# anonymousauthors001/SGS-GNN

Measured on AMD Instinct MI355X. Metric: sampled edges/sec + training steps/sec, Reddit hybrid 20% sparsity, higher is better.
Workload: dtype f32

## Files before the change

include/sgs_hip.h:

```cpp
#ifndef SGS_HIP_H_
#define SGS_HIP_H_

#include <stddef.h>
#include <stdint.h>

#ifdef __cplusplus
extern "C" {
#endif

#define SGS_ABI_VERSION 1

#define SGS_OK 0
#define SGS_EINVAL (-1)
#define SGS_EWORKSPACE (-2)
#define SGS_EHIP (-3)

typedef void* sgs_stream_t;

int sgs_abi_version(void);
const char* sgs_last_error(void);

int sgs_rng_set_epoch_buffer(const uint64_t* epoch_dev);
int sgs_exp_noise(uint64_t seed, uint64_t stream_id, int64_t E, float* noise, sgs_stream_t stream);
int sgs_dropout_keep(uint64_t seed, uint32_t site, int64_t rows, int64_t cols, float p, uint8_t* keep,
// ... 111 lines not shown
                          float* Hn, sgs_stream_t stream);
int sgs_gcn_norm_bwd_edge(const float* gw_hat, const float* gloop, int64_t n_edges, int64_t N, const float* dis,
                          const int32_t* loop_eid, const int64_t* edge_index, const float* Hn, float* dw,
                          sgs_stream_t stream);

#define SGS_ACT_NONE 0
#define SGS_ACT_RELU 1
#define SGS_ACT_RELU_DROPOUT 2
int sgs_spmm_csr(const float* X, int64_t N, int64_t D, int64_t nnz, const int32_t* ptr, const int32_t* col, const float* val,
                 const float* diag, const float* bias, int act, float p_drop, uint64_t seed, uint32_t site, float* Y,
                 sgs_stream_t stream);

int sgs_sddmm_csr(const float* A, const float* B, int64_t N, int64_t D, int64_t nnz, const int32_t* ptr, const int32_t* col,
                  const int32_t* eid, float* g, float* gdiag, sgs_stream_t stream);

int sgs_spmm_csr_variant(int64_t N, int64_t D, int64_t nnz, int aligned16);
int sgs_sddmm_csr_variant(int64_t N, int64_t D, int64_t nnz, int aligned16);

int sgs_spmm_long_rows_set(int on);
int sgs_spmm_long_rows_threshold(void);
int sgs_spmm_long_rows_active(int64_t N, int64_t D);

int sgs_act_bwd(const float* dY, const float* Y, int64_t n, int act, float p_drop, float* dZ, sgs_stream_t stream);
size_t sgs_colsum_workspace_bytes(int64_t N, int64_t D);
int sgs_colsum(const float* A, int64_t N, int64_t D, float* out, void* ws, size_t ws_bytes, sgs_stream_t stream);
int sgs_act_bwd_colsum(const float* dY, const float* Y, int64_t N, int64_t D, int act, float p_drop, float* dZ, float* colsum, void* ws,
                       size_t ws_bytes, sgs_stream_t stream);

int sgs_colsum_variant(int64_t N, int64_t D, int fused_act);

int sgs_gcn_pair_ok(int64_t N, int64_t nnz, int64_t D);
int sgs_spmm_csr_next(const float* X, int64_t N, int64_t D, int64_t nnz, const int32_t* ptr, const int32_t* col, const float* val,
                      const float* diag, const float* bias, int act, float p_drop, uint64_t seed, uint32_t site, const float* Wn, int64_t Dn,
                      float* Y, float* Z, sgs_stream_t stream);
int sgs_spmm_csr_bwd_prev(const float* dZ, int64_t N, int64_t D, int64_t nnz, const int32_t* ptr, const int32_t* col, const float* val,
                          const float* diag, const float* W, int64_t Dp, const float* Yp, int act, float p_drop, float* dX, float* dZp,
                          float* colsum, sgs_stream_t stream);

int sgs_gcn_dual_ok(int64_t N, int64_t nnz_a, int64_t nnz_b, int64_t D, int64_t Dn);
int sgs_spmm_csr_next_dual(const float* X, int64_t N, int64_t D, const float* bias, int act, float p_drop, uint32_t site, const float* Wn,
                           int64_t Dn, int64_t nnz_a, const int32_t* ptr_a, const int32_t* col_a, const float* val_a, const float* diag_a,
                           uint64_t seed_a, float* Y_a, float* Z_a, int64_t nnz_b, const int32_t* ptr_b, const int32_t* col_b,
                           const float* val_b, const float* diag_b, uint64_t seed_b, float* Y_b, float* Z_b, sgs_stream_t stream);
int sgs_spmm_csr_dual(const float* X_a, const float* X_b, int64_t N, int64_t D, const float* bias, int act, float p_drop, uint32_t site,
                      int64_t nnz_a, const int32_t* ptr_a, const int32_t* col_a, const float* val_a, const float* diag_a, uint64_t seed_a,
                      float* Y_a, int64_t nnz_b, const int32_t* ptr_b, const int32_t* col_b, const float* val_b, const float* diag_b,
                      uint64_t seed_b, float* Y_b, sgs_stream_t stream);

size_t sgs_edge_score_workspace_bytes(int64_t N, int64_t H, int64_t E);
int sgs_edge_score_hidden_supported(int64_t H);
int sgs_edge_score_get_variant(void);
int sgs_edge_score_get_bwd_variant(void);
void sgs_edge_score_set_bwd_variant(int variant);
int sgs_edge_score_bwd_tile(void);
void sgs_edge_score_set_variant(int variant);
int sgs_edge_score_fwd(const float* codes, const float* U, int64_t N, int64_t H, const int64_t* edge_index, int64_t E,
                       int64_t edge_id_offset, const float* W1, const float* b1, const float* w2, const float* b2,
                       float p_drop, uint64_t seed, uint32_t site, float* p_out, void* ws, size_t ws_bytes,
                       sgs_stream_t stream);
size_t sgs_edge_mates_workspace_bytes(int64_t n_edges);
int sgs_edge_mates(const int64_t* edge_index, int64_t n_edges, int64_t N, const int32_t* out_ptr, const int32_t* out_dst,
                   const int32_t* out_eid, int32_t* mate, void* ws, size_t ws_bytes, sgs_stream_t stream);
int sgs_edge_score_paired_supported(int64_t H);
int sgs_edge_score_fwd_paired(const float* codes, const float* U, int64_t N, int64_t H, const int64_t* edge_index, int64_t E,
                              int64_t edge_id_offset, const int32_t* canon, int64_t M, const int32_t* mate, const float* W1, const float* b1,
                              const float* w2, const float* b2, float p_drop, uint64_t seed, uint32_t site, float* p_out, void* ws,
                              size_t ws_bytes, sgs_stream_t stream);
int sgs_edge_score_bwd_core(const float* codes, const float* U, int64_t N, int64_t H, const int64_t* edge_index,
                            int64_t E, int64_t edge_id_offset, const int64_t* active_eid, int64_t n_active, const float* grad_p,
                            const float* W1, const float* b1, const float* w2, const float* b2, float p_drop,
                            uint64_t seed, uint32_t site, float* dv, float* hdz_part, float* dz, float* feat, void* ws,
                            size_t ws_bytes, sgs_stream_t stream);
int sgs_edge_score_bwd_dfeat_supported(int64_t H);
int sgs_edge_score_bwd_dfeat(const float* dv, int64_t n, int64_t H, const float* W1, float* dfeat, void* ws, size_t ws_bytes,
                             sgs_stream_t stream);

int sgs_edge_score_bwd_bits_supported(int64_t H);
int sgs_edge_score_fwd_mask(const float* codes, const float* U, int64_t N, int64_t H, const int64_t* edge_index, int64_t E,
                            int64_t edge_id_offset, const int32_t* canon, int64_t M, const int32_t* mate, const float* W1, const float* b1,
                            const float* w2, const float* b2, float p_drop, uint64_t seed, uint32_t site, float* p_out, uint32_t* maskbits,
                            void* ws, size_t ws_bytes, sgs_stream_t stream);
int sgs_edge_score_bwd_prep(const float* codes, int64_t N, int64_t H, const int64_t* edge_index, int64_t E, const int64_t* active_eid,
                            int64_t n_active, const float* grad_p, const float* p, const uint32_t* maskbits, float* dz, uint32_t* dvbits,
                            float* feat, sgs_stream_t stream);
int sgs_edge_score_dw2_from_parts(const float* W1, const float* T_raw, const float* U, const float* R_raw, const float* b1, const float* c_raw,
                                  int64_t N, int64_t H, float p_drop, float* dw2, sgs_stream_t stream);
int sgs_edge_score_probe_set(int stagger, int prio, uint32_t mode_mask);
int sgs_edge_score_probe_trace(unsigned long long* buf);
size_t sgs_edge_score_epd_workspace_bytes(int64_t H);
int sgs_edge_score_epd_fwd(const float* A, int64_t N, int64_t H, const int64_t* edge_index, int64_t E, int64_t edge_id_offset, const float* W1,
                           const float* b1, const float* w2, const float* b2, float p_hidden, uint64_t seed, uint32_t site, float p_ep,
                           uint64_t seed_x, uint32_t site_x, uint64_t seed_y, uint32_t site_y, float* p_out, void* ws, size_t ws_bytes,
                           sgs_stream_t stream);
int sgs_edge_score_epd_bwd_core(const float* A, int64_t N, int64_t H, const int64_t* edge_index, int64_t E, int64_t edge_id_offset,
                                const int64_t* active_eid, int64_t n_active, const float* grad_p, const float* W1, const float* b1, const float* w2,
                                const float* b2, float p_hidden, uint64_t seed, uint32_t site, float p_ep, uint64_t seed_x, uint32_t site_x,
                                uint64_t seed_y, uint32_t site_y, float* dv, float* hdz_part, float* dz, float* feat2, void* ws, size_t ws_bytes,
                                sgs_stream_t stream);
int sgs_edge_score_epd_reduce(const float* dfeat2, const float* A, int64_t N, int64_t H, const int32_t* in_ptr, const int32_t* in_src,
                              const int32_t* in_eid, const int32_t* out_ptr, const int32_t* out_dst, const int32_t* out_eid,
                              const int64_t* active_eid, int64_t edge_id_offset, float p_ep, uint64_t seed_x, uint32_t site_x, uint64_t seed_y,
                              uint32_t site_y, float* dA, sgs_stream_t stream);

int sgs_edge_score_bwd_prep_sd(const float* codes, int64_t N, int64_t H, const int64_t* edge_index, int64_t E, const int64_t* active_eid,
                               int64_t n_active, const float* grad_p, const float* p, const uint32_t* maskbits, float* dz, uint32_t* dvbits,
                               int32_t* sd, sgs_stream_t stream);
// ... 376 lines not shown
```

sgs-gnn_amd/csrc/edge_score.hip:

```cpp
#include <type_traits>

#include "sgs_common.h"
#include "endpoint_reduce.h"

namespace sgs {
namespace {

constexpr int kT = 256;
constexpr int kBM = 64;
constexpr int kBK = 16;
using f32x16 = __attribute__((ext_vector_type(16))) float;

__global__ void __launch_bounds__(kT) transpose_w1a(const float* __restrict__ W1, int H, float* __restrict__ WaT) {
    __shared__ float t[32][33];
    const int bx = blockIdx.x * 32, by = blockIdx.y * 32;
    const int tx = threadIdx.x & 31, ty = threadIdx.x >> 5;
    for (int r = ty; r < 32; r += 8) {
        const int h = by + r, k = bx + tx;
        t[r][tx] = (h < H && k < H) ? W1[static_cast<int64_t>(h) * 2 * H + k] : 0.f;
    }
    __syncthreads();
    for (int r = ty; r < 32; r += 8) {
        const int k = bx + r, h = by + tx;
        if (k < H && h < H) WaT[static_cast<int64_t>(k) * H + h] = t[tx][r];
// ... 890 lines not shown
    uint32_t p[3][4];
#pragma unroll
    for (int m = 0; m < 4; ++m) {
        float w0 = TRANSPOSED ? W1[static_cast<int64_t>(k0 + 2 * m) * 2 * H + h] : W1[static_cast<int64_t>(h) * 2 * H + k0 + 2 * m];
        float w1 = TRANSPOSED ? W1[static_cast<int64_t>(k0 + 2 * m + 1) * 2 * H + h] : W1[static_cast<int64_t>(h) * 2 * H + k0 + 2 * m + 1];
        if (TRANSPOSED && rowscale) { w0 *= rowscale[k0 + 2 * m] * scale; w1 *= rowscale[k0 + 2 * m + 1] * scale; }
        split3(w0, w1, p[0][m], p[1][m], p[2][m]);
    }
    uint4* o = Wp16 + (static_cast<int64_t>(kc) * NTl + t) * P * 64 + lane;
#pragma unroll
    for (int c = 0; c < P; ++c) o[c * 64] = make_uint4(p[c][0], p[c][1], p[c][2], p[c][3]);
}
inline int64_t pack_w1a_threads(int64_t H) { return (H / 16) * (H / 32) * 64; }

template <bool TRANSPOSED = false, int P = 3>
__global__ void __launch_bounds__(kT) pack_w1a_bf16x3(const float* __restrict__ W1, int H, uint4* __restrict__ Wp16,
                                                     const float* __restrict__ rowscale = nullptr, float scale = 1.f) {
    pack_w1a_bf16x3_one<TRANSPOSED, P>(static_cast<int64_t>(blockIdx.x) * kT + threadIdx.x, W1, H, Wp16, rowscale, scale);
}

template <bool SALU_MASK = false>
__device__ __forceinline__ uint32_t shift_in_bit(uint32_t acc, uint64_t mask) {
    uint32_t out;
    uint64_t carry_out;
    if constexpr (SALU_MASK) {
        asm("v_addc_co_u32_e64 %0, %1, %2, %2, %3" : "=v"(out), "=s"(carry_out) : "v"(acc), "s"(mask));
        return out;
    }
    asm("s_nop 1\n\tv_addc_co_u32_e64 %0, %1, %2, %2, %3" : "=v"(out), "=s"(carry_out) : "v"(acc), "s"(mask));
    return out;
}

#ifndef SGS_PHASE_PROBE
#define SGS_PHASE_PROBE 0
#endif
#if SGS_PHASE_PROBE
#define SGS_PHASE_STAMP(on, k, pre) do { if (on) asm volatile(pre "s_memtime %0\n\ts_waitcnt lgkmcnt(0)" : "=s"(pst[k]) :: "memory"); } while (0)
#define SGS_PHASE_BARRIER() do { if (!(a.prio & 4)) __syncthreads(); } while (0)
#else
#define SGS_PHASE_STAMP(on, k, pre) do { (void)(on); } while (0)
#define SGS_PHASE_BARRIER() __syncthreads()
#endif
#define SGS_STAMP(k) do { if (a.trace && tid == 0) a.trace[8 * blockIdx.x + (k)] = __builtin_readcyclecounter(); } while (0)

template <int NT, int NW, int MODE = 0, int NP = 3>
__global__ void __launch_bounds__(64 * NW, 8 / NW) edge_score_bf16x6_kernel(ScoreArgs a, const uint4* __restrict__ Wp16) {
    constexpr bool BWD = MODE == 1, FUSED = MODE == 5, GEMMB = MODE == 4 || MODE == 5, GEMM = MODE == 2 || GEMMB, PAIR = MODE == 3;
    constexpr bool ONE = NP == 1;
    static_assert(NP == 3 || (ONE && MODE != 1 && MODE != 2), "the one-piece form exists for MODEs 0, 3, 4 and 5");
    constexpr int H = 32 * NT;
    constexpr int NPH = H / 16;
    constexpr int CH = NT * NP * 64;
    constexpr int TH = 64 * NW;
    constexpr int SPT = CH / TH;
    static_assert(CH % TH == 0 && (ONE ? (SPT == 1 || SPT == 2) : (SPT == 3 || SPT == 6)), "unsupported shape");
    __shared__ uint4 wl[2][CH];
    __shared__ __attribute__((aligned(16))) float bw[2][H];
    const int tid = threadIdx.x, lane = tid & 63, wave = tid >> 6;
    const int kh = lane >> 5, l31 = lane & 31;
    const int64_t row0 = static_cast<int64_t>(blockIdx.x) * (32 * NW);
    if (a.dyn_n) {
        const int64_t live_n = *a.dyn_n;
        if (live_n < a.n) a.n = live_n;
        if (row0 >= a.n) return;
    }
    if (a.stagger > 0 && blockIdx.x >= 256 && blockIdx.x < 512 && a.n >= static_cast<int64_t>(1024) * 32 * NW)
        for (int w = 0; w < a.stagger; ++w) __builtin_amdgcn_s_sleep(1);
    if ((a.prio & 3) == 1) __builtin_amdgcn_s_setprio(1);
    SGS_STAMP(0);
    if (a.trace && tid == 0) {
        uint32_t hw, xcc;
        asm volatile("s_getreg_b32 %0, hwreg(HW_REG_HW_ID)" : "=s"(hw));
        asm volatile("s_getreg_b32 %0, hwreg(HW_REG_XCC_ID)" : "=s"(xcc));
        a.trace[8 * blockIdx.x + 4] = (static_cast<unsigned long long>(xcc) << 32) | hw;
    }
    if (!GEMM)
        for (int i = tid; i < H; i += TH) {
            bw[0][i] = a.b1[i];
            bw[1][i] = (!BWD && a.use_drop) ? a.w2[i] * a.drop_scale : a.w2[i];
        }
    const int64_t r = row0 + 32 * wave + l31;
    const bool live = r < a.n;
    int s = 0, d = 0;
    int64_t eg_id = 0;
    if (live && !GEMM) {
        eg_id = PAIR ? static_cast<int64_t>(a.canon[r]) : (a.active ? a.active[r] : r);
        s = static_cast<int>(a.src[eg_id]);
        d = static_cast<int>(a.dst[eg_id]);
    }
    const int64_t xrow = GEMM ? (live ? r : 0) : static_cast<int64_t>(s);
    const float4* xp = reinterpret_cast<const float4*>(a.codes + xrow * H + 8 * kh);
    const float4* yp = reinterpret_cast<const float4*>(a.codes + static_cast<int64_t>(d) * H + 8 * kh);

    f32x16 acc[NT];
#pragma unroll
    for (int t = 0; t < NT; ++t)
#pragma unroll
        for (int q = 0; q < 16; ++q) acc[t][q] = 0.f;

    const uint8_t* bp = GEMMB ? reinterpret_cast<const uint8_t*>(a.inbits + (live ? r : 0) * (H / 32)) + kh : nullptr;
    struct Feat { float4 xa, xb, ya, yb; uint32_t mb; };
    const uint32_t wl_lds = static_cast<uint32_t>(reinterpret_cast<uintptr_t>((__attribute__((address_space(3))) void*)(&wl[0][0])));
    const uint32_t wave_u = __builtin_amdgcn_readfirstlane(wave);
    const uint32_t voff = static_cast<uint32_t>(tid) * 16u;
    auto dma_one = [&](int ph, int stage, int k) {
        const uint4* gb = Wp16 + static_cast<int64_t>(ph) * CH + k * TH;
        const uint32_t ld = wl_lds + static_cast<uint32_t>((stage * CH + k * TH) * 16) + wave_u * 1024u;
        asm volatile("s_mov_b32 m0, %1\n\ts_nop 0\n\tglobal_load_lds_dwordx4 %0, %2" :: "v"(voff), "s"(ld), "s"(gb) : "memory");
    };
    auto dma = [&](int ph, int stage) {
#pragma unroll
        for (int k = 0; k < SPT; ++k) dma_one(ph, stage, k);
    };
    auto fload_x = [&](int kc, Feat& f) {
        if constexpr (GEMMB) { f.mb = bp[2 * kc]; return; }
        f.xa = xp[4 * kc]; f.xb = xp[4 * kc + 1];
    };
    auto fload_y = [&](int kc, Feat& f) {
        if constexpr (!GEMM) { f.ya = yp[4 * kc]; f.yb = yp[4 * kc + 1]; }
    };
    auto fload = [&](int kc, Feat& f) { fload_x(kc, f); fload_y(kc, f); };
    struct WF { uint4 q1, q2, q3; };
    Feat fa;
    dma(0, 0);
    fload(0, fa);
    asm volatile("s_waitcnt vmcnt(0)" ::: "memory");
    __syncthreads();
    SGS_STAMP(1);
    struct Pieces { u32x4 F1, F2, F3; };
    struct SplitState { float a, b; uint32_t p1; float4 pa, pb; };
    auto split_slot = [&](int slot, Feat& f, int kc_, bool wr, Pieces& P, SplitState& st) {
        const int j = slot >> 1;
        if constexpr (GEMMB) {
            if (slot != 0) return;
            const uint32_t b = f.mb;
#pragma unroll
            for (int m = 0; m < 4; ++m) P.F1[m] = ((b >> (2 * m)) & 1u ? 0x3F80u : 0u) | ((b >> (2 * m + 1)) & 1u ? 0x3F800000u : 0u);
            P.F2 = P.F1; P.F3 = P.F1;
        } else if constexpr (ONE) {
            const float4 x = slot < 2 ? f.xa : f.xb, y = slot < 2 ? f.ya : f.yb;
            const float x0 = (slot & 1) ? x.z : x.x, x1 = (slot & 1) ? x.w : x.y, y0 = (slot & 1) ? y.z : y.x, y1 = (slot & 1) ? y.w : y.y;
            P.F1[slot] = pk_bf16(x0 * y0, x1 * y1);
        } else {
            if ((slot & 1) == 0) {
                const float4 x = j < 2 ? f.xa : f.xb, y = j < 2 ? f.ya : f.yb;
                const float x0 = (j & 1) ? x.z : x.x, x1 = (j & 1) ? x.w : x.y, y0 = (j & 1) ? y.z : y.x, y1 = (j & 1) ? y.w : y.y;
                st.a = GEMM ? x0 : x0 * y0;
                st.b = GEMM ? x1 : x1 * y1;
                if constexpr (BWD) {
                    float4& pp = j < 2 ? st.pa : st.pb;
                    if (j & 1) { pp.z = st.a; pp.w = st.b; } else { pp.x = st.a; pp.y = st.b; }
                    if ((j & 1) && live && wr) reinterpret_cast<float4*>(a.feat + r * H + 16 * kc_ + 8 * kh)[j >> 1] = pp;
                }
                const uint32_t p1 = pk_bf16(st.a, st.b);
                st.a -= __uint_as_float(p1 << 16);
                st.b -= __uint_as_float(p1 & 0xFFFF0000u);
                P.F1[j] = p1;
            } else {
                const uint32_t p2 = pk_bf16(st.a, st.b);
                st.a -= __uint_as_float(p2 << 16);
                st.b -= __uint_as_float(p2 & 0xFFFF0000u);
                P.F2[j] = p2;
                P.F3[j] = pk_bf16(st.a, st.b);
            }
        }
    };
    constexpr int kSlots = GEMMB ? 1 : (ONE ? 4 : 8);
    auto split_feat = [&](Feat& f, int kc_, bool wr, Pieces& P) {
        SplitState st;
#pragma unroll
        for (int q = 0; q < kSlots; ++q) split_slot(q, f, kc_, wr, P, st);
    };
#if SGS_PHASE_PROBE
    unsigned long long pst[8] = {0, 0, 0, 0, 0, 0, 0, 0};
#endif
    auto chunk = [&](const uint4* wcur, const uint4* wnx, int stage_next, WF& A, WF& B, WF& Cn, const Pieces& C, Pieces& Nx, Feat& f, int kc1,
                     int kn_, bool wr, bool tr) {
        const bf16x8 f1 = __builtin_bit_cast(bf16x8, C.F1), f2 = __builtin_bit_cast(bf16x8, C.F2), f3 = __builtin_bit_cast(bf16x8, C.F3);
// ... 28 lines not shown
            }
#pragma unroll
            for (int m = 0; m < kPerTile; ++m) {
                const int slot = t * kPerTile + m;
                if (t & 1) one(t, B, m); else one(t, A, m);
                if (slot < kSlots + 2 + SPT) {
                    __builtin_amdgcn_sched_barrier(0);
                    if (slot < kSlots) split_slot(slot, f, kc1, wr, Nx, st);
                    else if (slot == kSlots) fload_x(kn_, f);
                    else if (slot == kSlots + 1) fload_y(kn_, f);
                    else dma_one(kc1, stage_next, slot - kSlots - 2);
                    __builtin_amdgcn_sched_barrier(0);
                }
            }
            if (t + 2 < NT) { if (t & 1) wload(wcur, t + 2, B); else wload(wcur, t + 2, A); }
            __builtin_amdgcn_sched_barrier(0);
        }
    };
    constexpr int kFL = GEMMB ? 1 : 4;
    auto chunk1 = [&](const uint4* wcur, const uint4* wnx, int stage_next, WF& A, WF& B, WF& Cn, const Pieces& C, Pieces& Nx, Feat& fs, int kc1,
                      int kn_) {
        const bf16x8 f1 = __builtin_bit_cast(bf16x8, C.F1);
        auto wload = [&](const uint4* wsrc, int t, WF& w) { w.q1 = wsrc[t * 64 + lane]; };
        constexpr int kItems = kSlots + SPT + 2, kPer = (kItems + NT - 2) / (NT - 1);
        SplitState st;
#pragma unroll
        for (int t = 0; t < NT; ++t) {
            if (t == NT - 1) {
                static_assert(kFL == 1 || kFL == 4, "the wait below names the count");
                if constexpr (kFL == 1) asm volatile("s_waitcnt vmcnt(1)" ::: "memory");
                else                    asm volatile("s_waitcnt vmcnt(4)" ::: "memory");
                SGS_PHASE_BARRIER();
                wload(wnx, 0, A);
                wload(wnx, 1, Cn);
                __builtin_amdgcn_sched_barrier(0);
            }
            acc[t] = __builtin_amdgcn_mfma_f32_32x32x16_bf16(__builtin_bit_cast(bf16x8, (t & 1) ? B.q1 : A.q1), f1, acc[t], 0, 0, 0);
#pragma unroll
            for (int q = 0; q < kPer; ++q) {
                const int it = t * kPer + q;
                if (t < NT - 1 && it < kItems) {
                    __builtin_amdgcn_sched_barrier(0);
                    if (it < kSlots) split_slot(it, fs, kc1, false, Nx, st);
                    else if (it < kSlots + SPT) dma_one(kc1, stage_next, it - kSlots);
                    else if (it == kSlots + SPT) fload_x(kn_, fs);
                    else fload_y(kn_, fs);
                    __builtin_amdgcn_sched_barrier(0);
                }
            }
            if (t + 2 < NT) { if (t & 1) wload(wcur, t + 2, B); else wload(wcur, t + 2, A); }
            __builtin_amdgcn_sched_barrier(0);
        }
    };
    Pieces pc, pn_;
    WF wa, wb, wc;
    {
        const uint4* w0 = wl[0];
        if constexpr (ONE) {
            wa.q1 = w0[lane]; wb.q1 = w0[64 + lane];
        } else {
            wa.q1 = w0[lane]; wa.q2 = w0[64 + lane]; wa.q3 = w0[128 + lane];
            wb.q1 = w0[192 + lane]; wb.q2 = w0[256 + lane]; wb.q3 = w0[320 + lane];
        }
    }
    split_feat(fa, 0, true, pc);
    fload(NPH > 1 ? 1 : 0, fa);
    static_assert(NPH % 2 == 0, "the phase loop is unrolled by two (the odd fragment set and the operand pieces alternate)");
    if constexpr (ONE) {
        Feat fb;
        fload(2, fb);
#pragma unroll 1
        for (int ph = 0; ph < NPH; ph += 2) {
            chunk1(wl[0], wl[1], 1, wa, wb, wc, pc, pn_, fa, ph + 1, ph + 3 < NPH ? ph + 3 : NPH - 1);
            chunk1(wl[1], wl[0], 0, wa, wc, wb, pn_, pc, fb, ph + 2 < NPH ? ph + 2 : NPH - 1, ph + 4 < NPH ? ph + 4 : NPH - 1);
        }
        asm volatile("s_waitcnt vmcnt(0)" ::: "memory");
    } else
#pragma unroll 1
    for (int ph = 0; ph < NPH; ph += 2) {
        const bool tr = a.trace != nullptr && ph == NPH / 2;
        SGS_PHASE_STAMP(tr, 0, "");
        chunk(wl[0], wl[1], 1, wa, wb, wc, pc, pn_, fa, ph + 1, ph + 2 < NPH ? ph + 2 : NPH - 1, true, tr);
        SGS_PHASE_STAMP(tr, 4, "");
        chunk(wl[1], wl[0], 0, wa, wc, wb, pn_, pc, fa, ph + 2 < NPH ? ph + 2 : NPH - 1, ph + 3 < NPH ? ph + 3 : NPH - 1, ph + 2 < NPH, false);
    }
#if SGS_PHASE_PROBE
    if (a.trace && lane == 0)
        for (int k = 0; k < 5; ++k) a.trace[8 * (static_cast<int64_t>(gridDim.x) + 4 * blockIdx.x + wave) + k] = pst[k];
#endif
    __syncthreads();
    if constexpr (FUSED) {
        const float rs = live ? a.indz[r] : 0.f;
        int sr = 0, dr = 0;
        if (live) { sr = a.sd[2 * r]; dr = a.sd[2 * r + 1]; }
        const int nxt = __shfl(sr, (lane & 32) | ((l31 + 1) & 31), 64);
        const bool endrow = live && (l31 == 31 || r + 1 >= a.n || nxt != sr);
        const uint32_t endmask = static_cast<uint32_t>(__ballot(endrow && kh == 0));
        constexpr int LS = 68;
        constexpr bool kInWl = sizeof(wl) >= static_cast<size_t>(NW) * 32 * LS * sizeof(float);
        __shared__ float ot_own[kInWl ? 1 : NW * 32 * LS];
        float* ot = (kInWl ? reinterpret_cast<float*>(&wl[0][0]) : ot_own) + wave * (32 * LS);
        const float* cs = a.codes + static_cast<int64_t>(sr) * H + 4 * kh;
        const float* cd = a.codes + static_cast<int64_t>(dr) * H + 4 * kh;
        const int64_t wrow = (row0 + 32 * wave) >> 5;
        float4 s4n[8], d4n[8];
#pragma unroll
        for (int ii = 0; ii < 8; ++ii) {
            s4n[ii] = *reinterpret_cast<const float4*>(cs + 8 * ii);
            d4n[ii] = *reinterpret_cast<const float4*>(cd + 8 * ii);
        }
#pragma unroll
        for (int Q = 0; Q < NT / 2; ++Q) {
#pragma unroll
            for (int ii = 0; ii < 8; ++ii) {
                const int i = 8 * Q + ii, t = i >> 2, g4 = i & 3;
                const float4 s4 = s4n[ii], d4 = d4n[ii];
                const float f0 = rs * acc[t][4 * g4], f1 = rs * acc[t][4 * g4 + 1], f2 = rs * acc[t][4 * g4 + 2], f3 = rs * acc[t][4 * g4 + 3];
                if (live) *reinterpret_cast<float4*>(a.feat + r * H + 8 * i + 4 * kh) = make_float4(f0 * s4.x, f1 * s4.y, f2 * s4.z, f3 * s4.w);
                *reinterpret_cast<float4*>(ot + l31 * LS + 8 * ii + 4 * kh) = make_float4(f0 * d4.x, f1 * d4.y, f2 * d4.z, f3 * d4.w);
            }
            if (Q + 1 < NT / 2) {
#pragma unroll
                for (int ii = 0; ii < 8; ++ii) {
                    s4n[ii] = *reinterpret_cast<const float4*>(cs + 8 * (8 * (Q + 1) + ii));
                    d4n[ii] = *reinterpret_cast<const float4*>(cd + 8 * (8 * (Q + 1) + ii));
                }
            }
            __builtin_amdgcn_fence(__ATOMIC_RELEASE, "wavefront");
            __builtin_amdgcn_wave_barrier();
            __builtin_amdgcn_fence(__ATOMIC_ACQUIRE, "wavefront");
            float col[32];
#pragma unroll
            for (int row = 0; row < 32; ++row) col[row] = ot[row * LS + lane];
            float run = 0.f;
#pragma unroll
            for (int row = 0; row < 32; ++row) {
                run += col[row];
                if ((endmask >> row) & 1u) {
                    const int64_t slot = wrow + __builtin_amdgcn_readlane(sr, row);
                    a.opart[slot * H + 64 * Q + lane] = run;
                    run = 0.f;
                }
            }
            __builtin_amdgcn_fence(__ATOMIC_RELEASE, "wavefront");
            __builtin_amdgcn_wave_barrier();
            __builtin_amdgcn_fence(__ATOMIC_ACQUIRE, "wavefront");
        }
        return;
    }
    if constexpr (GEMM) {
        if (live) {
            const float rs = GEMMB ? a.indz[r] : 1.f;
#pragma unroll
            for (int i = 0; i < 4 * NT; ++i)
                *reinterpret_cast<float4*>(a.feat + r * H + 8 * i + 4 * kh) =
                    GEMMB ? make_float4(rs * acc[i >> 2][4 * (i & 3)], rs * acc[i >> 2][4 * (i & 3) + 1], rs * acc[i >> 2][4 * (i & 3) + 2],
                                        rs * acc[i >> 2][4 * (i & 3) + 3])
                          : make_float4(acc[i >> 2][4 * (i & 3)], acc[i >> 2][4 * (i & 3) + 1], acc[i >> 2][4 * (i & 3) + 2], acc[i >> 2][4 * (i & 3) + 3]);
        }
        return;
    }

    constexpr int kPF = BWD ? 8 : (PAIR ? 5 : 6);
    __builtin_amdgcn_s_waitcnt(0);
    __builtin_amdgcn_sched_barrier(0);
    const int Hrt = a.H;
    const uint32_t rkey = dropout_row_key(fold_epoch(a.seed, a.epoch), a.site, static_cast<uint64_t>(a.row_offset + eg_id));
    int64_t mate_id = -1;
    uint32_t rkey2 = 0u;
    float z2 = 0.f;
    if constexpr (PAIR) {
        if (live) mate_id = a.mate[eg_id];
        rkey2 = dropout_row_key(fold_epoch(a.seed, a.epoch), a.site, static_cast<uint64_t>(a.row_offset + (mate_id >= 0 ? mate_id : 0)));
    }
    const float* Us = a.U + static_cast<int64_t>(s) * H + 4 * kh;
    const float* Ud = a.U + static_cast<int64_t>(d) * H + 4 * kh;
    float4 us[kPF], ud[kPF];
    if constexpr (BWD) {
#pragma unroll
        for (int i = 0; i < kPF; ++i) {
            us[i] = *reinterpret_cast<const float4*>(Us + 8 * i);
            ud[i] = *reinterpret_cast<const float4*>(Ud + 8 * i);
        }
    }
    if constexpr (!BWD) {
        if ((a.prio & 3) == 1) __builtin_amdgcn_s_setprio(0);
        if ((a.prio & 3) == 2) __builtin_amdgcn_s_setprio(2);
        SGS_STAMP(2);
        const bool want_bits = a.dvbits != nullptr;
        const bool use_drop = a.use_drop != 0;
        const uint32_t thr = a.drop_thresh;
        float zA[2] = {0.f, 0.f}, zB[2] = {0.f, 0.f};
        uint32_t fb[NT], fb2[PAIR ? NT : 1];
#pragma unroll
        for (int t = 0; t < NT; ++t) fb[t] = 0u;
#pragma unroll
        for (int t = 0; t < (PAIR ? NT : 1); ++t) fb2[t] = 0u;
#pragma unroll
        for (int k = 0; k < kPF; ++k) {
            us[k] = *reinterpret_cast<const float4*>(Us + 8 * (4 * NT - 1 - k));
// ... 688 lines not shown
    const size_t sm = score_smem_bytes(NT);
#define SGS_SCORE_CASE(NT_)                                                                                        \
    do {                                                                                                            \
        static bool raised = false;                                                                                 \
        if (!raised) {                                                                                              \
            SGS_HIP_OK(hipFuncSetAttribute(reinterpret_cast<const void*>(&edge_score_kernel<NT_, BWD, EPD>),        \
                                           hipFuncAttributeMaxDynamicSharedMemorySize, static_cast<int>(sm)));      \
            raised = true;                                                                                          \
        }                                                                                                           \
        hipLaunchKernelGGL((edge_score_kernel<NT_, BWD, EPD>), grid, blk, sm, stream, a);                           \
    } while (0)
    switch (NT) {
        case 2: SGS_SCORE_CASE(2); break;
        case 4: SGS_SCORE_CASE(4); break;
        default: SGS_SCORE_CASE(8); break;
    }
#undef SGS_SCORE_CASE
    SGS_LAUNCH_OK();
    return SGS_OK;
}

inline bool hidden_ok(int64_t H) { return (H >= 4 && H <= 256 && H % 4 == 0) || (H > 256 && H <= 1024 && H % 32 == 0); }

template <bool BWD, bool EPD, bool PAIRED = false>
int launch_score_wide(const ScoreArgs& a, hipStream_t stream) {
    hipLaunchKernelGGL((edge_score_wide_kernel<BWD, EPD, PAIRED>), dim3(static_cast<unsigned>(cdiv(a.n, kBM))), dim3(kT), 0, stream, a);
    SGS_LAUNCH_OK();
    return SGS_OK;
}

inline int check_common(const char* who, int64_t N, int64_t H, int64_t E, float p_drop) {
    SGS_REQUIRE(N >= 0 && E >= 0 && N < (int64_t(1) << 31), SGS_EINVAL, "%s: bad sizes", who);
    SGS_REQUIRE(hidden_ok(H), SGS_EINVAL,
                "%s: hidden size H=%lld unsupported (need 4 <= H <= 256 with H %% 4 == 0, or 256 < H <= 1024 with H %% 32 == 0)", who, (long long)H);
    SGS_REQUIRE(p_drop >= 0.f && p_drop < 1.f, SGS_EINVAL, "%s: bad dropout probability", who);
    return SGS_OK;
}

}
}

using namespace sgs;

static int g_probe_stagger = -1;
static int g_probe_prio = 0;
static unsigned g_stagger_modes = (1u << 0) | (1u << 3);
static unsigned long long* g_probe_trace = nullptr;
static void bf16x6_launch_knobs(ScoreArgs& a, int mode, int64_t H, int P = 3) {
    a.stagger = (g_stagger_modes >> mode) & 1u ? (g_probe_stagger >= 0 ? g_probe_stagger : static_cast<int>(80 * (H / 32)) / (P == 3 ? 1 : 6)) : 0;
    a.prio = g_probe_prio;
    a.trace = g_probe_trace;
}

template <int MODE, int P>
static int launch_bf16x6(ScoreArgs& a, const uint4* Wp16, int64_t rows, int64_t H, hipStream_t stream, size_t dyn_lds = 0) {
    bf16x6_launch_knobs(a, MODE, H, P);
    const dim3 grid(static_cast<unsigned>(cdiv(rows, 128))), blk(256);
    if (H == 256) hipLaunchKernelGGL((edge_score_bf16x6_kernel<8, 4, MODE, P>), grid, blk, dyn_lds, stream, a, Wp16);
    else          hipLaunchKernelGGL((edge_score_bf16x6_kernel<4, 4, MODE, P>), grid, blk, 0, stream, a, Wp16);
    SGS_LAUNCH_OK();
    return SGS_OK;
}

static void score_args(ScoreArgs& a, const float* codes, const float* U, const int64_t* edge_index, int64_t E, const int64_t* active, int64_t n,
                       int64_t edge_id_offset, int64_t H, const float* WaT, const float* b1, const float* w2, const float* b2, float p_drop,
                       uint64_t seed, uint32_t site) {
    a.codes = codes; a.U = U; a.src = edge_index; a.dst = edge_index + E; a.active = active; a.n = n; a.row_offset = edge_id_offset;
    a.H = static_cast<int>(H); a.WaT = WaT; a.b1 = b1; a.w2 = w2; a.b2 = b2;
    a.drop_scale = 1.0f / (1.0f - p_drop); a.drop_thresh = dropout_thresh(p_drop); a.seed = seed; a.epoch = epoch_ptr(); a.site = site;
    a.use_drop = p_drop > 0.f;
}

struct ScoreWs {
    float* WaT;
    float* Ceo;
    float* zpart;
    unsigned int* ctr;
    uint4* Wp16;
    size_t end;
};
static ScoreWs carve_score_ws(void* ws, int64_t N, int64_t H, int64_t E) {
    Carver cv(ws);
    ScoreWs w;
    w.WaT = cv.take<float>(static_cast<size_t>(H) * H);
    w.Ceo = cv.take<float>(static_cast<size_t>(N) * H);
    w.zpart = cv.take<float>(2 * static_cast<size_t>(E));
    w.ctr = cv.take<unsigned int>(64);
    w.Wp16 = reinterpret_cast<uint4*>(cv.take<uint64_t>(static_cast<size_t>(H) * H));
    w.end = cv.off;
    return w;
}
static uint4* fused_wp16(void* ws, int64_t H) { return carve_score_ws(ws, 0, H, 0).Wp16; }

static void launch_transpose_w1a(const float* W1, int64_t H, float* WaT, hipStream_t stream) {
    hipLaunchKernelGGL(transpose_w1a, dim3(cdiv(H, 32), cdiv(H, 32)), dim3(kT), 0, stream, W1, static_cast<int>(H), WaT);
}

static void launch_pack_stream(const float* W1, int64_t H, float* WaT, const float* codes, int64_t N, float* Ceo, hipStream_t stream) {
    const int n_w = static_cast<int>(cdiv(H * H, kT));
    hipLaunchKernelGGL(pack_stream_operands, dim3(static_cast<unsigned>(n_w + cdiv(N * H, kT))), dim3(kT), 0, stream, W1, static_cast<int>(H), WaT,
                       n_w, codes, N, Ceo);
}

template <bool TRANSPOSED>
static void launch_pack_w1a(int P, const float* W1, int64_t H, uint4* Wp16, hipStream_t stream, const float* rowscale = nullptr, float scale = 1.f) {
    const dim3 grid(static_cast<unsigned>(cdiv(pack_w1a_threads(H), kT)));
    if (P == 1) hipLaunchKernelGGL((pack_w1a_bf16x3<TRANSPOSED, 1>), grid, dim3(kT), 0, stream, W1, static_cast<int>(H), Wp16, rowscale, scale);
    else        hipLaunchKernelGGL((pack_w1a_bf16x3<TRANSPOSED, 3>), grid, dim3(kT), 0, stream, W1, static_cast<int>(H), Wp16, rowscale, scale);
}

#define SGS_LAUNCH_ROWBLOCK(K16_, K4_, ...)                                                    \
    do {                                                                                       \
        if (nnz >= 64 * N) hipLaunchKernelGGL(K16_, grid, dim3(1024), 0, stream, __VA_ARGS__); \
        else               hipLaunchKernelGGL(K4_, grid, dim3(256), 0, stream, __VA_ARGS__);   \
    } while (0)

extern "C" {

size_t sgs_edge_score_workspace_bytes(int64_t N, int64_t H, int64_t E) {
    return carve_score_ws(nullptr, N < 0 ? 0 : N, H < 0 ? 0 : H, E < 0 ? 0 : E).end + 256;
}

static int g_score_variant = -1;
static int g_bwd_variant = -1;
void sgs_edge_score_set_variant(int v) { g_score_variant = v; }
void sgs_edge_score_set_bwd_variant(int v) { g_bwd_variant = v; }
int sgs_edge_score_get_variant(void) { return g_score_variant; }
int sgs_edge_score_get_bwd_variant(void) { return g_bwd_variant; }
int sgs_edge_score_bwd_tile(void) { return kBM; }

int sgs_edge_score_fwd(const float* codes, const float* U, int64_t N, int64_t H, const int64_t* edge_index, int64_t E,
                       int64_t edge_id_offset, const float* W1, const float* b1, const float* w2, const float* b2, float p_drop,
                       uint64_t seed, uint32_t site, float* p_out, void* ws, size_t ws_bytes, sgs_stream_t stream_) {
    hipStream_t stream = static_cast<hipStream_t>(stream_);
    if (int rc = check_common("sgs_edge_score_fwd", N, H, E, p_drop)) return rc;
    if (E == 0) return SGS_OK;
    SGS_REQUIRE(codes && U && edge_index && W1 && b1 && w2 && b2 && p_out, SGS_EINVAL, "sgs_edge_score_fwd: null pointer");
    SGS_REQUIRE(ws && ws_bytes >= sgs_edge_score_workspace_bytes(N, H, E), SGS_EWORKSPACE, "sgs_edge_score_fwd: workspace too small");
    const ScoreWs w = carve_score_ws(ws, N, H, E);
    float* const WaT = w.WaT;
    float* const Ceo = w.Ceo;
    ScoreArgs a{};
    score_args(a, codes, U, edge_index, E, nullptr, E, edge_id_offset, H, WaT, b1, w2, b2, p_drop, seed, site);
    a.p_out = p_out;
    a.dyn_n = dyn_edges_ptr();
    if (H > 256) {
        SGS_REQUIRE(N > 0, SGS_EINVAL, "sgs_edge_score_fwd: edges without nodes");
        launch_transpose_w1a(W1, H, WaT, stream);
        return launch_score_wide<false, false>(a, stream);
    }
    int variant = g_score_variant;
    if (variant < 0) variant = (cdiv(E, kBM2) >= 512) ? (H % 128 == 0 ? 4 : 3) : 1;
    if (variant == 2 && a.dyn_n) variant = 3;
    if (variant == 2 && H % 64 == 0 && N > 0) {
        float* const zpart = w.zpart;
        unsigned int* const ctr = w.ctr;
        if (int rc = zero_async(ctr, 256, stream)) return rc;
        launch_pack_stream(W1, H, WaT, codes, N, Ceo, stream);
        constexpr int TH = 768;
        const size_t sm = static_cast<size_t>(H / 2) * H * 4;
        const int64_t n_tiles = cdiv(E, 32);
        int64_t nwg = 256;
        if (nwg > 2 * cdiv(n_tiles, TH / 64)) nwg = 2 * cdiv(n_tiles, TH / 64);
        if (nwg < 2) nwg = 2;
#define SGS_WRES_CASE(NT_)                                                                                              \
        do {                                                                                                                \
            static bool raised = false;                                                                                     \
            if (!raised) {                                                                                                  \
                SGS_HIP_OK(hipFuncSetAttribute(reinterpret_cast<const void*>(&edge_score_wres_kernel<NT_, TH>),            \
                                               hipFuncAttributeMaxDynamicSharedMemorySize, static_cast<int>(sm)));          \
                raised = true;                                                                                              \
            }                                                                                                               \
            hipLaunchKernelGGL((edge_score_wres_kernel<NT_, TH>), dim3(static_cast<unsigned>(nwg)), dim3(TH), sm, stream, a, WaT, Ceo, \
                               ctr, zpart);                                                                                 \
        } while (0)
        if (H == 256) SGS_WRES_CASE(8); else if (H == 128) SGS_WRES_CASE(4); else SGS_WRES_CASE(2);
#undef SGS_WRES_CASE
        hipLaunchKernelGGL(edge_score_finish, dim3(cdiv(E, kT)), dim3(kT), 0, stream, zpart, E, b2, p_out);
        SGS_LAUNCH_OK();
        return SGS_OK;
    }
// ... 542 lines not shown
```

Measured before the change: 112.3 million.

## Add 8-wave dfeat GEMM variant using packed mask bits and dynamic LDS

Adds an 8-wave (512-thread) variant of the bf16x6 edge-score kernel for GEMM-B modes at H=256. Each phase stages twice the weight chunk in dynamic LDS. Instead of loading float features, it reads packed keep-mask bits (inbits) and expands them into bf16 0/1 operands. By default it is selected for mode 4 with at least 65536 rows, and a setter lets callers override it. The aim is to raise weight reuse per block and cut feature-load traffic, at the cost of higher LDS use and lower occupancy per CU.

```diff
diff --git a/include/sgs_hip.h b/include/sgs_hip.h
--- a/include/sgs_hip.h
+++ b/include/sgs_hip.h
@@ -187,6 +187,7 @@
 int sgs_edge_score_get_variant(void);
 int sgs_edge_score_get_bwd_variant(void);
 void sgs_edge_score_set_bwd_variant(int variant);
+int sgs_edge_score_set_dfeat_variant(int variant);
 int sgs_edge_score_bwd_tile(void);
 void sgs_edge_score_set_variant(int variant);
 int sgs_edge_score_fwd(const float* codes, const float* U, int64_t N, int64_t H, const int64_t* edge_index, int64_t E,
diff --git a/sgs-gnn_amd/csrc/edge_score.hip b/sgs-gnn_amd/csrc/edge_score.hip
--- a/sgs-gnn_amd/csrc/edge_score.hip
+++ b/sgs-gnn_amd/csrc/edge_score.hip
@@ -966,9 +966,15 @@
     constexpr int NPH = H / 16;
     constexpr int CH = NT * NP * 64;
     constexpr int TH = 64 * NW;
-    constexpr int SPT = CH / TH;
-    static_assert(CH % TH == 0 && (ONE ? (SPT == 1 || SPT == 2) : (SPT == 3 || SPT == 6)), "unsupported shape");
-    __shared__ uint4 wl[2][CH];
+    constexpr bool WIDE = NW == 8;
+    static_assert(!WIDE || (GEMMB && NP == 3 && NT == 8), "the 8-wave shape exists for MODEs 4 and 5 at NP = 3, H = 256");
+    constexpr int ST = WIDE ? 2 * CH : CH;
+    constexpr int SPT = ST / TH;
+    static_assert(ST % TH == 0 && (ONE ? (SPT == 1 || SPT == 2) : (SPT == 3 || SPT == 6)), "unsupported shape");
+    __shared__ uint4 wl_own[WIDE ? 1 : 2][WIDE ? 1 : CH];
+    extern __shared__ uint4 wl_dyn[];
+    uint4 (*wl)[ST];
+    if constexpr (WIDE) wl = reinterpret_cast<uint4 (*)[ST]>(wl_dyn); else wl = wl_own;
     __shared__ __attribute__((aligned(16))) float bw[2][H];
     const int tid = threadIdx.x, lane = tid & 63, wave = tid >> 6;
     const int kh = lane >> 5, l31 = lane & 31;
@@ -1018,8 +1024,8 @@
     const uint32_t wave_u = __builtin_amdgcn_readfirstlane(wave);
     const uint32_t voff = static_cast<uint32_t>(tid) * 16u;
     auto dma_one = [&](int ph, int stage, int k) {
-        const uint4* gb = Wp16 + static_cast<int64_t>(ph) * CH + k * TH;
-        const uint32_t ld = wl_lds + static_cast<uint32_t>((stage * CH + k * TH) * 16) + wave_u * 1024u;
+        const uint4* gb = Wp16 + static_cast<int64_t>(ph) * ST + k * TH;
+        const uint32_t ld = wl_lds + static_cast<uint32_t>((stage * ST + k * TH) * 16) + wave_u * 1024u;
         asm volatile("s_mov_b32 m0, %1\n\ts_nop 0\n\tglobal_load_lds_dwordx4 %0, %2" :: "v"(voff), "s"(ld), "s"(gb) : "memory");
     };
     auto dma = [&](int ph, int stage) {
@@ -1036,8 +1042,10 @@
     auto fload = [&](int kc, Feat& f) { fload_x(kc, f); fload_y(kc, f); };
     struct WF { uint4 q1, q2, q3; };
     Feat fa;
+    const uint32_t* mwp = WIDE ? a.inbits + (live ? r : 0) * (H / 32) : nullptr;
+    uint32_t mw = 0u;
     dma(0, 0);
-    fload(0, fa);
+    if constexpr (WIDE) mw = mwp[0]; else fload(0, fa);
     asm volatile("s_waitcnt vmcnt(0)" ::: "memory");
     __syncthreads();
     SGS_STAMP(1);
@@ -1172,6 +1180,50 @@
             __builtin_amdgcn_sched_barrier(0);
         }
     };
+    auto mask_piece = [&](uint32_t b) {
+        u32x4 f;
+#pragma unroll
+        for (int m = 0; m < 4; ++m) f[m] = ((b >> (2 * m)) & 1u ? 0x3F80u : 0u) | ((b >> (2 * m + 1)) & 1u ? 0x3F800000u : 0u);
+        return f;
+    };
+    auto phase2 = [&](const uint4* wcur, const uint4* wnx, int stage_next, WF& A, WF& B, WF& Cn, const u32x4& C0, const u32x4& C1, u32x4& N0,
+                      u32x4& N1, int pn, int pl, bool tr) {
+        const bf16x8 f0 = __builtin_bit_cast(bf16x8, C0), f1 = __builtin_bit_cast(bf16x8, C1);
+        auto wload = [&](const uint4* wsrc, int u, WF& w) {
+            w.q1 = wsrc[(u * 3 + 0) * 64 + lane];
+            w.q2 = wsrc[(u * 3 + 1) * 64 + lane];
+            w.q3 = wsrc[(u * 3 + 2) * 64 + lane];
+        };
+#pragma unroll
+        for (int u = 0; u < 2 * NT; ++u) {
+            if (u == 2 * NT - 1) {
+                SGS_PHASE_STAMP(tr, 1, "s_waitcnt lgkmcnt(0)\n\t");
+                asm volatile("s_waitcnt vmcnt(0)" ::: "memory");
+                SGS_PHASE_STAMP(tr, 2, "");
+                SGS_PHASE_BARRIER();
+                SGS_PHASE_STAMP(tr, 3, "");
+                wload(wnx, 0, A);
+                wload(wnx, 1, Cn);
+                __builtin_amdgcn_sched_barrier(0);
+            }
+#pragma unroll
+            for (int m = 0; m < 3; ++m) {
+                const WF& w = (u & 1) ? B : A;
+                const bf16x8 wm = __builtin_bit_cast(bf16x8, m == 0 ? w.q3 : m == 1 ? w.q2 : w.q1);
+                acc[u % NT] = __builtin_amdgcn_mfma_f32_32x32x16_bf16(wm, u < NT ? f0 : f1, acc[u % NT], 0, 0, 0);
+                const int slot = 3 * u + m;
+                if (slot < 2 + SPT) {
+                    __builtin_amdgcn_sched_barrier(0);
+                    if (slot == 0) { N0 = mask_piece(mw >> (8 * kh)); N1 = mask_piece(mw >> (16 + 8 * kh)); }
+                    else if (slot == 1) mw = mwp[pl];
+                    else dma_one(pn, stage_next, slot - 2);
+                    __builtin_amdgcn_sched_barrier(0);
+                }
+            }
+            if (u + 2 < 2 * NT) { if (u & 1) wload(wcur, u + 2, B); else wload(wcur, u + 2, A); }
+            __builtin_amdgcn_sched_barrier(0);
+        }
+    };
     Pieces pc, pn_;
     WF wa, wb, wc;
     {
@@ -1183,10 +1235,25 @@
             wb.q1 = w0[192 + lane]; wb.q2 = w0[256 + lane]; wb.q3 = w0[320 + lane];
         }
     }
-    split_feat(fa, 0, true, pc);
-    fload(NPH > 1 ? 1 : 0, fa);
+    if constexpr (!WIDE) {
+        split_feat(fa, 0, true, pc);
+        fload(NPH > 1 ? 1 : 0, fa);
+    }
     static_assert(NPH % 2 == 0, "the phase loop is unrolled by two (the odd fragment set and the operand pieces alternate)");
-    if constexpr (ONE) {
+    if constexpr (WIDE) {
+        constexpr int NPH2 = NPH / 2;
+        static_assert(NPH2 % 2 == 0 && NPH2 >= 2, "unrolled by two, as below");
+        u32x4 c0 = mask_piece(mw >> (8 * kh)), c1 = mask_piece(mw >> (16 + 8 * kh)), n0, n1;
+        mw = mwp[1];
+#pragma unroll 1
+        for (int ph = 0; ph < NPH2; ph += 2) {
+            const bool tr = a.trace != nullptr && ph == NPH2 / 2;
+            SGS_PHASE_STAMP(tr, 0, "");
+            phase2(wl[0], wl[1], 1, wa, wb, wc, c0, c1, n0, n1, ph + 1, ph + 2 < NPH2 ? ph + 2 : NPH2 - 1, tr);
+            SGS_PHASE_STAMP(tr, 4, "");
+            phase2(wl[1], wl[0], 0, wa, wc, wb, n0, n1, c0, c1, ph + 2 < NPH2 ? ph + 2 : NPH2 - 1, ph + 3 < NPH2 ? ph + 3 : NPH2 - 1, false);
+        }
+    } else if constexpr (ONE) {
         Feat fb;
         fload(2, fb);
 #pragma unroll 1
@@ -1206,7 +1273,8 @@
     }
 #if SGS_PHASE_PROBE
     if (a.trace && lane == 0)
-        for (int k = 0; k < 5; ++k) a.trace[8 * (static_cast<int64_t>(gridDim.x) + 4 * blockIdx.x + wave) + k] = pst[k];
+        for (int k = 0; k < 5; ++k) a.trace[8 * (static_cast<int64_t>(gridDim.x) + NW * blockIdx.x + wave) + k] = pst[k];
+    if constexpr (FUSED) SGS_STAMP(2);
 #endif
     __syncthreads();
     if constexpr (FUSED) {
@@ -1217,7 +1285,7 @@
         const bool endrow = live && (l31 == 31 || r + 1 >= a.n || nxt != sr);
         const uint32_t endmask = static_cast<uint32_t>(__ballot(endrow && kh == 0));
         constexpr int LS = 68;
-        constexpr bool kInWl = sizeof(wl) >= static_cast<size_t>(NW) * 32 * LS * sizeof(float);
+        constexpr bool kInWl = 2 * ST * sizeof(uint4) >= static_cast<size_t>(NW) * 32 * LS * sizeof(float);
         __shared__ float ot_own[kInWl ? 1 : NW * 32 * LS];
         float* ot = (kInWl ? reinterpret_cast<float*>(&wl[0][0]) : ot_own) + wave * (32 * LS);
         const float* cs = a.codes + static_cast<int64_t>(sr) * H + 4 * kh;
@@ -1266,6 +1334,9 @@
             __builtin_amdgcn_wave_barrier();
             __builtin_amdgcn_fence(__ATOMIC_ACQUIRE, "wavefront");
         }
+#if SGS_PHASE_PROBE
+        SGS_STAMP(3);
+#endif
         return;
     }
     if constexpr (GEMM) {
@@ -2060,8 +2131,28 @@
     a.trace = g_probe_trace;
 }
 
+static int g_dfeat_variant = -1;
+static bool dfeat_wide_selected(int mode, int64_t rows) { return g_dfeat_variant < 0 ? (mode == 4 && rows >= 65536) : g_dfeat_variant == 1; }
+
+template <int MODE>
+static int launch_dfeat_wide(ScoreArgs& a, const uint4* Wp16, int64_t rows, hipStream_t stream) {
+    constexpr size_t lds = 2 * 2 * (8 * 3 * 64) * sizeof(uint4);
+    bf16x6_launch_knobs(a, MODE, 256, 3);
+    static bool raised = false;
+    if (!raised) {
+        SGS_HIP_OK(hipFuncSetAttribute(reinterpret_cast<const void*>(&edge_score_bf16x6_kernel<8, 8, MODE, 3>),
+                                       hipFuncAttributeMaxDynamicSharedMemorySize, static_cast<int>(lds)));
+        raised = true;
+    }
+    hipLaunchKernelGGL((edge_score_bf16x6_kernel<8, 8, MODE, 3>), dim3(static_cast<unsigned>(cdiv(rows, 256))), dim3(512), lds, stream, a, Wp16);
+    SGS_LAUNCH_OK();
+    return SGS_OK;
+}
+
 template <int MODE, int P>
 static int launch_bf16x6(ScoreArgs& a, const uint4* Wp16, int64_t rows, int64_t H, hipStream_t stream, size_t dyn_lds = 0) {
+    if constexpr ((MODE == 4 || MODE == 5) && P == 3)
+        if (H == 256 && dfeat_wide_selected(MODE, rows)) return launch_dfeat_wide<MODE>(a, Wp16, rows, stream);
     bf16x6_launch_knobs(a, MODE, H, P);
     const dim3 grid(static_cast<unsigned>(cdiv(rows, 128))), blk(256);
     if (H == 256) hipLaunchKernelGGL((edge_score_bf16x6_kernel<8, 4, MODE, P>), grid, blk, dyn_lds, stream, a, Wp16);
@@ -2135,6 +2226,11 @@
 void sgs_edge_score_set_bwd_variant(int v) { g_bwd_variant = v; }
 int sgs_edge_score_get_variant(void) { return g_score_variant; }
 int sgs_edge_score_get_bwd_variant(void) { return g_bwd_variant; }
+int sgs_edge_score_set_dfeat_variant(int v) {
+    const int prev = g_dfeat_variant;
+    g_dfeat_variant = v < 0 ? -1 : (v != 0);
+    return prev;
+}
 int sgs_edge_score_bwd_tile(void) { return kBM; }
 
 int sgs_edge_score_fwd(const float* codes, const float* U, int64_t N, int64_t H, const int64_t* edge_index, int64_t E,
```

Measured after the change: 112.7 million, median of 6. No clear change (+0.3%).
